# Ascend-Research/HeadPoseEstimation-WHENet

Hardware: AMD Instinct MI355X
Metric: head crops/sec (224x224) (higher is better)
Workload: dtype f16

## Files before the change

### headposeestimation-whenet_amd/csrc/capi.cpp

```cpp
#include <algorithm>
#include <chrono>
#include <cstdio>
#include <cstring>
#include <fstream>
#include <memory>
#include <mutex>
#include <new>
#include <exception>
#include <string>
#include <thread>
#include <utility>
#include <vector>

#include "engine.h"
#include "engine_internal.h"

constexpr int MAX_INFLIGHT_ENGINES = 4;
struct whenet_ctx {
    whenet::Engine* engine = nullptr;
    std::vector<whenet::Engine*> replicas;
    std::vector<char> snapshot;
    int device_id = 0, dtype = WHENET_F32;
    int inflight = 1;
    size_t next = 0;
// ... 1212 lines not shown
        std::memcpy(out, v, sizeof(v));
        return WHENET_OK;
    } catch (...) {
        return WHENET_EINVAL;
    }
}

int whenet_front2_static_check(int row, int field, int delta) {
    try {
        return whenet::front2_static_selftest(row, field, delta) == 0 ? WHENET_OK : WHENET_EINVAL;
    } catch (...) {
        return WHENET_EINVAL;
    }
}

int whenet_front_static_check(int row, int field, int delta) {
    try {
        return whenet::front_static_selftest(row, field, delta) == 0 ? WHENET_OK : WHENET_EINVAL;
    } catch (...) {
        return WHENET_EINVAL;
    }
}

int whenet_pw_static_check(int row, int field, int delta) {
    try {
        return whenet::pw_static_selftest(row, field, delta) == 0 ? WHENET_OK : WHENET_EINVAL;
    } catch (...) {
        return WHENET_EINVAL;
    }
}
// ... 21 lines not shown
```

### headposeestimation-whenet_amd/csrc/engine.cpp

```cpp
#include "engine_internal.h"

#include <mutex>

#include <algorithm>
#include <cstdlib>
#include <cmath>
#include <cstring>

namespace whenet {

using namespace detail;

void* Engine::upload_bytes(const void* p, size_t nbytes) {
    weight_allocs_.emplace_back();
    weight_allocs_.back().reset(nbytes);
    void* d = weight_allocs_.back().as<void>();
    if (nbytes) WHENET_HIP_CHECK(hipMemcpy(d, p, nbytes, hipMemcpyHostToDevice));
    return d;
}

template <typename T> T* Engine::upload(const std::vector<T>& v) {
    return static_cast<T*>(upload_bytes(v.data(), v.size() * sizeof(T)));
}

// ... 211 lines not shown
        WHENET_REQUIRE(split_ || value == 0, WHENET_EINVAL, "split_pw: the handle was not created as WHENET_F32S");
        split_pw_ = value != 0;
    } else if (key == "detector_dtype") {
        WHENET_REQUIRE(value == 0 || value == 1, WHENET_EINVAL, "detector_dtype must be 0 (binary16 storage, default) or 1 (float32)");
        const int dtype = value == 1 ? WHENET_F32 : WHENET_F16;
        WHENET_REQUIRE(det_ == nullptr || dtype == det_dtype_, WHENET_EINVAL,
                       "detector_dtype: a detector is attached and its weights were packed when it was loaded: set the option on a "
                       "handle without a detector, then load again");
        det_dtype_ = dtype;
        return;
    } else if (key == "host_pinned_max") {
        WHENET_REQUIRE(value >= 0 && value <= 4096, WHENET_EINVAL, "host_pinned_max must be 0..4096");
        sync();
        host_pinned_max_ = int(value);
        return;
    } else if (key == "se_fuse_tiny") {
        WHENET_REQUIRE(value >= 0 && value <= 64, WHENET_EINVAL, "se_fuse_tiny must be 0..64");
        se_fuse_tiny_ = int(value);
    } else if (key == "letterbox_cache") {
        WHENET_REQUIRE(value >= 1 && value <= 32, WHENET_EINVAL, "letterbox_cache must be 1..32");
        sync();
        lb_cache_.clear();
        lb_cache_cap_ = int(value);
        return;
    } else if (key == "jpeg_entropy") {
        WHENET_REQUIRE(value >= 0 && value <= 2, WHENET_EINVAL, "jpeg_entropy must be 0 (an interval per lane), 1 (segmented) or 2 (auto, default)");
        jpeg_entropy_ = int(value);
        return;
    } else if (key == "jpeg_seg_lanes") {
        WHENET_REQUIRE(value == 0 || value == 16 || value == 32 || value == 64, WHENET_EINVAL, "jpeg_seg_lanes must be 0 (default), 16, 32 or 64");
// ... 168 lines not shown
    } else {
        const DevBlock& c = blocks_[size_t(index)];
        const BlockSchedule cs = block_schedule(c);
        if (cs.use_mb7 || !cs.use_f7) return false;
        if (c.spec.has_skip() && c.project.K < 320) return false;
    }
    static constexpr bool WINS[17] = {false, false, false, false, false, false, false, false, false, false, false, false,
                                      true, true, true, true, true};
    return act_layout_ == 2 || (index <= 16 && WINS[index]);
}

bool Engine::front2_static(int index) const {
    static constexpr bool WINS[17] = {false, false, true, true, true, true, false, true, true, true, true, true, true,
                                      false, false, false, false};
    return front2_static_ && index >= 0 && index <= 16 && WINS[index];
}

bool Engine::pw_static(int index) const {
    static constexpr bool WINS[17] = {false, false, true, true, true, false, false, true, false, true, false, false, false,
                                      true, true, true, true};
    return pw_static_ && se_fuse_ == 1 && index >= 0 && index <= 16 && WINS[index];
}

bool Engine::front_static(int index) const {
    static constexpr bool WINS[17] = {false, false, false, false, false, false, true, false, false, false, false, false, false,
                                      false, false, false, false};
    return front_static_ && index >= 0 && index <= 16 && WINS[index];
}

void* Engine::enqueue_blocks(int first, int last, const View& v, void* cur, int n, hipStream_t s, LaunchRecorder* rec,
// ... 109 lines not shown
        fill_front_tiled(a, b);
        a.wep = b.expand.wp;
        a.wdt = b.dw.wt;
        if (fold == 2) {
            a.wep = d_fold12_w32_;
            a.be = fold12_pw_.bias;
            a.Cin = fold12_pw_.K;
            a.KSe = fold12_pw_.KS;
            a.NTe = fold12_pw_.NTILES;
            a.in_gate = static_cast<const float*>(v.gate);
        }
        a.xcd_grouped = xcd_grouped(1, n);
        a.plan = b.f2plan;
        a.plan.threads = front2_threads(b.f2plan, n);
        a.static_form = front2_static(sp.index);
        R(p + "/front", "front",
          kernel_name_front2(sp.k, sp.s, a.KSe, a.plan.threads, a.plan.xs, a.in_gate != nullptr, front2_static_row(a)).c_str(),
          bytes(a.Cin), flops(a.Cin), [&] { launch_front2(a, s); });
    } else if (bs.use_f2s) {
        Front2sArgs a{};
        fill_front_common(a, b, v, in, n);
        fill_front_tiled(a, b);
        a.weps = b.expand.wps;
        a.wdt = b.dw.wts;
        a.KSe = b.expand.KSs;
        a.wsi = b.expand.wsi;
        a.wsi_d = b.dw.wts_wsi;
        a.tm = b.f2s_tm;
        a.plan = b.f2splan;
        R(p + "/front", "front", kernel_name_front2s(sp.k, sp.s, a.KSe, a.plan.threads, a.tm, false).c_str(), bytes(a.Cin),
          flops(a.Cin), [&] { launch_front2s(a, s); });
    } else {
// ... 594 lines not shown
```

### headposeestimation-whenet_amd/csrc/engine.h

```cpp
#pragma once

#include <deque>
#include <map>
#include <memory>
#include <string>
#include <tuple>
#include <utility>
#include <vector>

#include "common.h"
#include "kernels.h"
#include "snapshot.h"

namespace whenet {

template <typename H, hipError_t (*Destroy)(H)>
class Owned {
  public:
    Owned() = default;
    Owned(Owned&& o) noexcept : h_(o.h_) { o.h_ = nullptr; }
    ~Owned() { reset(); }
    void reset() {
        if (h_) (void)Destroy(h_);
        h_ = nullptr;
// ... 344 lines not shown
                         hipStream_t s, LaunchRecorder* rec, bool in_blocked, bool out_blocked);
    template <typename A> void fill_front_common(A& a, const DevBlock& b, const View& v, const void* in, int n) const;
    Head7Args head7_args(const void* x, float* feat, int n) const;
    PwArgs head_pw_args(const void* x, void* out, int n) const { return pw_args(head_, x, out, n * 49, 49, ACT_SWISH); }
    void* enqueue_blocks(int first, int last, const View& v, void* cur, int n, hipStream_t s, LaunchRecorder* rec,
                         bool b1_dw_done = false);
    bool stem_fuse_active() const;
    bool fold12_active() const;
    bool head_fused() const;
    bool heads_split_active() const;
    void launch_heads_stage(const HeadsArgs& h, const View& v, hipStream_t s);
    bool act_blocked(int index) const;
    bool front_static(int index) const;
    bool pw_static(int index) const;
    bool front2_static(int index) const;
    int act_layout_ = 1;
    struct BlockSchedule {
        bool fused = false, use_f2 = false, use_f2s = false, use_f7 = false, se_in_front = false, se_fused = false, se_mfma = false;
        bool use_mb7 = false;
        int se_ntiles = 1, se_chunks = 1;
    };
    BlockSchedule block_schedule(const DevBlock& b, int n = 0) const;
    int se_fuse_tiny_ = 0;
    int f2s_mask_ = -1;
    bool single_stage_call_ = false;
    bool range_call_ = false;
    int lanes_for(int n, int want) const;
    template <typename F> void for_each_lane(int n, int lanes, hipStream_t s, F&& body);
    void enqueue_lanes(const uint8_t* d_in, int n, Results out, hipStream_t s, int want = 0);
    void run_forward(const uint8_t* d_in, int n, Results out, hipStream_t s, int want = 0);
// ... 71 lines not shown
    int se_fuse_ = 1;
    int front_impl_ = 1;
    bool poison_ = false;
    bool head_fuse_ = true;
    bool front7_ = true;
    bool mb7_ = false;
    int xcd_map_ = 7;
    bool xcd_always_ = false;
    bool xcd_grouped(int bit, int n) const {
        return (xcd_map_ & bit) != 0 && (xcd_always_ || n >= 128);
    }
    bool stem_fuse_ = true;
    bool front_static_ = true;
    bool pw_static_ = true;
    bool front2_static_ = true;
    bool fold12_ = true;
    int lanes_ = 2;
    bool lane_graphs_ = false;
    int min_lane_crops_ = 16;
    int host_lanes_ = 2;
    Stream stream_, copy_stream_;
    std::vector<Stream> lane_streams_;
    std::vector<Event> join_ev_;
    Event fork_ev_;
    hipDeviceProp_t prop_{};
    int64_t params_backbone_ = 0, params_heads_ = 0;
    int n_tensors_ = 0;

    std::vector<DeviceBuffer> weight_allocs_;
    float *d_lut_ = nullptr, *d_stem_w_ = nullptr, *d_stem_b_ = nullptr;
// ... 59 lines not shown
```

### headposeestimation-whenet_amd/csrc/front2.hip

```cpp
#include "device_math.h"
#include "kernels.h"
#include "stamps.h"

#include <atomic>
#include <cstdlib>
#include <string>
#include <vector>

namespace whenet {

namespace {

constexpr int RL = 7;

__device__ __forceinline__ int fdiv2(int q, float rinv) { return int((float(q) + 0.5f) * rinv); }

struct F2Params {
    const half_t* x;
    const half_t* wep;
    const float* be;
    const half_t* wdt;
    const float* bd;
    half_t* out;
    float* rpart;
    const float* w1t;
    const float* in_gate;
    int H, Ho, Cin, Cexp, pad, NTe;
    int CC, TH, TXG, tiles_x, EH, EWp, RP, CP;
    int off_stage, off_red, off_sum;
    int R, RPse;
    int ntiles, chunks, n, xcd;
};

struct Tuned2 { int k, s, H, Cexp, CC, TH, TXG, xs, use, threads; };
constexpr Tuned2 TUNED2[] = {
#include "front2_tuned.inc"
};
constexpr int NTUNED2 = int(sizeof(TUNED2) / sizeof(TUNED2[0]));

struct F2Shape {
    int H, Ho, Cin, Cexp, pad, NTe;
    int CC, TH, TXG, tiles_x, tiles_y, EH, EWp, RP, CP;
    int off_stage, off_red, off_sum;
    int R, RPse;
    int ntiles, chunks;
    int k, s, xs, threads, KS, gated, lds_bytes;
};

constexpr int cdiv(int a, int b) { return (a + b - 1) / b; }

constexpr F2Shape f2_static_shape(int row) {
    const Tuned2 t = TUNED2[row];
    F2Shape g{};
// ... 38 lines not shown
#pragma unroll
    for (int qq = 0; qq < 4; ++qq) {
        if (!EDGE || (drd[qq] < nr_left && dcd[qq] < ng_left)) {
            const float2v y0 = swish2(float2v{acc[4 * qq], acc[4 * qq + 1]});
            const float2v y1 = swish2(float2v{acc[4 * qq + 2], acc[4 * qq + 3]});
            half4 o;
            o[0] = half_t(y0[0]);
            o[1] = half_t(y0[1]);
            o[2] = half_t(y1[0]);
            o[3] = half_t(y1[1]);
            *reinterpret_cast<half4*>(ep + eoff[qq]) = o;
        }
    }
}

template <int K, int S, int KS, int NTHR, int XS, bool GATED, int ROW>
__device__ __forceinline__ void front2_body(const F2Params p) {
    constexpr F2Shape sg = f2_static_shape(ROW < 0 ? 0 : ROW);
    static_assert(ROW < 0 || (sg.k == K && sg.s == S && sg.KS == KS && sg.threads == NTHR && sg.xs == XS && (sg.gated != 0) == GATED),
                  "front2: the static plan belongs to another instantiation");
#define GEO(f) (ROW >= 0 ? sg.f : p.f)
    constexpr bool ONE_TILE = ROW >= 0 && sg.CC <= 32;
    constexpr int NCH = (3 * S + K + XS + 3) / 4;
    constexpr int NER = (RL - 1) * S + K;
    constexpr int NWAVE = NTHR / 64;
    constexpr int PF = KS <= 7 ? KS : 6;

    extern __shared__ __attribute__((aligned(16))) unsigned char smem[];
    unsigned char* E = smem;

// ... 347 lines not shown
                    const int c = q + 4 * i;
                    if (c < ccur) accr = fmaf(s_sum[c], w1v[i], accr);
                }
                for (int c = q + 4 * W1V; c < ccur; c += 4) accr = fmaf(s_sum[c], wrow[c], accr);
            }
            const float pair = accr + quad_xor1(accr);
            const float tot = pair + quad_xor2(pair);
            if (q == 0)
                p.rpart[((size_t(b) * GEO(ntiles) + tile) * GEO(chunks) + chunk) * GEO(RPse) + jo] = (jo < GEO(R)) ? tot : 0.0f;
        }
    }
    STAMP(6);
}
#undef GEO

template <int K, int S, int KS, int NTHR, int XS, bool GATED>
__global__ __launch_bounds__(NTHR) void whenet_front2_kernel(const F2Params p) {
    front2_body<K, S, KS, NTHR, XS, GATED, -1>(p);
}

template <int K, int S, int KS, int NTHR, int XS, bool GATED, int ROW>
__global__ __launch_bounds__(NTHR) void whenet_front2_static_kernel(const F2Params p) {
    front2_body<K, S, KS, NTHR, XS, GATED, ROW>(p);
}

}

namespace {

constexpr bool f2_has_static(int row) { return TUNED2[row].use != 0; }

const char* f2_static_mismatch(const F2Shape& g, const Front2Args& a) {
    const Front2Plan& pl = a.plan;
    struct Field { const char* name; long long want, got; };
    const Field fields[] = {
        {"H", g.H, a.H}, {"Ho", g.Ho, a.Ho}, {"Cin", g.Cin, a.Cin}, {"Cexp", g.Cexp, a.Cexp}, {"pad", g.pad, a.pad}, {"NTe", g.NTe, a.NTe},
        {"CC", g.CC, pl.CC}, {"TH", g.TH, pl.TH}, {"TXG", g.TXG, pl.TXG}, {"tiles_x", g.tiles_x, pl.tiles_x}, {"tiles_y", g.tiles_y, pl.tiles_y},
        {"EH", g.EH, pl.EH}, {"EWp", g.EWp, pl.EWp}, {"RP", g.RP, pl.RP}, {"CP", g.CP, pl.CP},
// ... 20 lines not shown
        if (!f2_has_static(r)) continue;
        const F2Shape g = f2_static_shape(r);
        if (g.k == a.k && g.s == a.s && g.H == a.H && g.Ho == a.Ho && g.Cin == a.Cin && g.Cexp == a.Cexp && g.pad == a.pad && g.NTe == a.NTe &&
            g.KS == a.KSe && g.R == a.R && (g.gated != 0) == (a.in_gate != nullptr) && g.CC == a.plan.CC && g.TH == a.plan.TH &&
            g.TXG == a.plan.TXG && g.xs == a.plan.xs && g.threads == a.plan.threads)
            return r;
    }
    return -1;
}

void front2_static_check(int row, const Front2Args& a) {
    WHENET_REQUIRE(row >= 0 && row < NTUNED2 && f2_has_static(row), WHENET_EINVAL, "front2: no static form for this row of the plan table");
    f2_static_require(f2_static_shape(row), a);
}

int front2_static_selftest(int row, int field, int delta) {
    WHENET_REQUIRE(row >= 0 && row < NTUNED2 && f2_has_static(row), WHENET_EINVAL, "front2: no static form for this row of the plan table");
    WHENET_REQUIRE(field >= -1 && field < int(sizeof(F2Shape) / sizeof(int)), WHENET_EINVAL, "front2: no such field");
    F2Shape g = f2_static_shape(row);
    Front2Args a{};
    a.k = g.k;  a.s = g.s;  a.H = g.H;  a.Ho = g.Ho;  a.Cin = g.Cin;  a.Cexp = g.Cexp;  a.pad = g.pad;  a.NTe = g.NTe;  a.KSe = g.KS;  a.R = g.R;
    a.in_gate = g.gated ? reinterpret_cast<const float*>(&g) : nullptr;
    a.plan = make_front2_plan(g.k, g.s, g.Ho, g.Cexp, TUNED2[row].CC, TUNED2[row].TH, TUNED2[row].TXG, TUNED2[row].threads, TUNED2[row].xs);
    if (field >= 0) reinterpret_cast<int*>(&g)[field] += delta;
    f2_static_require(g, a);
    return 0;
}

namespace {

struct OncePerDevice {
    std::atomic<bool> done[64];
    OncePerDevice() { for (auto& d : done) d.store(false, std::memory_order_relaxed); }
};

template <int K, int S, int KS, int NTHR, int XS = 0, bool GATED = false, int ROW = -1>
void launch_f2(const Front2Args& a, hipStream_t stream) {
    const auto kernel = [] {
        if constexpr (ROW >= 0) return &whenet_front2_static_kernel<K, S, KS, NTHR, XS, GATED, ROW>;
        else return &whenet_front2_kernel<K, S, KS, NTHR, XS, GATED>;
    }();
    const Front2Plan& pl = a.plan;
    F2Params p{};
    p.x = static_cast<const half_t*>(a.x);
    p.wep = static_cast<const half_t*>(a.wep);
    p.be = a.be;
    p.wdt = static_cast<const half_t*>(a.wdt);
    p.bd = a.bd;
    p.out = static_cast<half_t*>(a.out);
    p.rpart = a.rpart;
    p.w1t = a.w1t;
    p.in_gate = a.in_gate;
    p.H = a.H;  p.Ho = a.Ho;  p.Cin = a.Cin;  p.Cexp = a.Cexp;  p.pad = a.pad;  p.NTe = a.NTe;
    p.CC = pl.CC;  p.TH = pl.TH;  p.TXG = pl.TXG;  p.tiles_x = pl.tiles_x;
    p.EH = pl.EH;  p.EWp = pl.EWp;  p.RP = pl.RP;  p.CP = pl.CP;
    p.off_stage = pl.off_stage;  p.off_red = pl.off_red;  p.off_sum = pl.off_sum;
    p.R = a.R;  p.RPse = (a.R + 3) & ~3;
    p.ntiles = pl.tiles_x * pl.tiles_y;  p.chunks = pl.chunks;  p.n = a.n;  p.xcd = a.xcd_grouped ? 1 : 0;
    WHENET_REQUIRE(pl.lds_bytes <= 160 * 1024, WHENET_EINVAL, "front2: the tile plan needs more than 160 KB of LDS");
    static OncePerDevice attr;
    int dev = 0;
    WHENET_HIP_CHECK(hipGetDevice(&dev));
    if (dev >= 0 && dev < 64 && !attr.done[dev].load(std::memory_order_acquire)) {
        if constexpr (ROW >= 0) front2_static_check(ROW, a);
        WHENET_HIP_CHECK(hipFuncSetAttribute(reinterpret_cast<const void*>(kernel), hipFuncAttributeMaxDynamicSharedMemorySize, 160 * 1024));
        attr.done[dev].store(true, std::memory_order_release);
    }
    hipLaunchKernelGGL(kernel, dim3(unsigned(pl.tiles_x * pl.tiles_y) * unsigned(pl.chunks) * unsigned(a.n)), dim3(NTHR),
                       pl.lds_bytes, stream, p);
    WHENET_HIP_CHECK(hipGetLastError());
}

void launch_f2_static(int row, const Front2Args& a, hipStream_t stream) {
    switch (row) {
        case 0: launch_f2<3, 2, 2, 512, 0, true, 0>(a, stream); break;
        case 1: launch_f2<3, 1, 2, 256, 0, false, 1>(a, stream); break;
        case 2: launch_f2<5, 2, 2, 256, 0, false, 2>(a, stream); break;
        case 3: launch_f2<5, 1, 3, 256, 0, false, 3>(a, stream); break;
        case 5: launch_f2<3, 1, 5, 256, 0, false, 5>(a, stream); break;
        case 6: launch_f2<5, 1, 5, 256, 0, false, 6>(a, stream); break;
        case 7: launch_f2<5, 1, 7, 256, 0, false, 7>(a, stream); break;
        case 8: launch_f2<5, 2, 7, 256, 0, false, 8>(a, stream); break;
        default: throw Error(WHENET_EINVAL, "front2: no static form for this row of the plan table");
    }
}

template <int NTHR>
void launch_f2_shape(const Front2Args& a, hipStream_t stream) {
// ... 113 lines not shown

void launch_front2(const Front2Args& a, hipStream_t stream) {
    WHENET_REQUIRE(a.KSe == ceil_div(a.Cin, 16), WHENET_EINVAL, "front2: k-steps do not match Cin");
    WHENET_REQUIRE(a.in_gate == nullptr || (a.k == 3 && a.s == 2 && a.KSe == 2 && a.Cin == 32), WHENET_EINVAL,
                   "front2: the gated-input form exists for the 3x3 / stride-2 / Cin = 32 shape only");
    Front2Args b = a;
    if (b.plan.threads != 256) {
        b.plan = make_front2_plan(a.k, a.s, a.Ho, a.Cexp, a.plan.CC, a.plan.TH, a.plan.TXG, a.plan.threads, a.plan.xs);
    }
    const int row = front2_static_row(b);
    if (row >= 0) launch_f2_static(row, b, stream);
    else if (b.plan.threads == 512) launch_f2_shape<512>(b, stream);
    else launch_f2_shape<256>(b, stream);
}

std::string kernel_name_front2(int k, int s, int kse, int threads, int xs, bool gated, int static_row) {
    return std::string(static_row >= 0 ? "whenet_front2_static_kernel<" : "whenet_front2_kernel<") + std::to_string(k) + ", " +
           std::to_string(s) + ", " + std::to_string(kse) + ", " + std::to_string(threads) + ", " + std::to_string(xs) + ", " +
           (gated ? "true" : "false") + (static_row >= 0 ? ", " + std::to_string(static_row) : std::string()) + ">";
}

}
```

### headposeestimation-whenet_amd/csrc/kernels.h

```cpp
#pragma once

#include <string>
#include <vector>

#include "common.h"
#include "overlay_host.h"
#include "jpeg_host.h"
#include "jpeg_dec_host.h"
#include "jpeg_dec_seg_host.h"

namespace whenet {

struct StemArgs {
    const uint8_t* in;
    void* out;
    const float* w;
    const float* bias;
    const float* lut;
    int n;
    const float* in_f32 = nullptr;
};
void launch_stem(const StemArgs& a, int dtype, hipStream_t stream);

struct DwPlan {
// ... 201 lines not shown
struct Front2Args {
    const void* x;
    const void* wep;
    const float* be;
    const void* wdt;
    const float* bd;
    void* out;
    float* rpart;
    const float* w1t;
    const float* in_gate;
    int R;
    int k, s, H, Ho, Cin, Cexp, pad, KSe, NTe, n;
    Front2Plan plan;
    bool xcd_grouped = false;
    bool static_form = false;
};
void launch_front2(const Front2Args& a, hipStream_t stream);
std::string kernel_name_front2(int k, int s, int kse, int threads, int xs, bool gated, int static_row = -1);
int front2_static_row(const Front2Args& a);
void front2_static_check(int row, const Front2Args& a);
int front2_static_selftest(int row, int field, int delta);

struct Front2sArgs {
    const void* x;
    const void* weps;
    const float* be;
    const void* wdt;
    const float* bd;
    void* out;
    float* rpart;
    const float* w1t;
    int R;
    int k, s, H, Ho, Cin, Cexp, pad, KSe, NTe, n;
    float wsi = 1.0f;
    float wsi_d = 1.0f;
    int tm = 2;
// ... 340 lines not shown
```

### headposeestimation-whenet_amd/whenet_hip/_lib.py

```python
from __future__ import annotations

import ctypes as C
import os
from typing import Optional

import numpy as np

ABI_VERSION = 6
F32, F16, F32S = 0, 1, 2
OK, ENOENT, EIO, ENOMEM, ENODEV, EINVAL, EFORMAT, EHIP = 0, -2, -5, -12, -19, -22, -74, -1000
EOVERFLOW = -75
MAX_INFLIGHT = 4

_HERE = os.path.dirname(os.path.abspath(__file__))
LIB_PATH = os.path.join(_HERE, "..", "lib", "libwhenet_hip.so")


class Info(C.Structure):
    _fields_ = [("abi_version", C.c_int32), ("dtype", C.c_int32), ("device_id", C.c_int32),
                ("compute_units", C.c_int32), ("params_backbone", C.c_int64),
                ("params_heads", C.c_int64), ("n_tensors", C.c_int32),
                ("n_kernels_per_forward", C.c_int32), ("macs_per_crop", C.c_int64),
                ("arena_bytes", C.c_int64), ("capacity", C.c_int32), ("graph_enabled", C.c_int32),
                ("device_name", C.c_char * 64), ("arch", C.c_char * 32)]
# ... 112 lines not shown
    "whenet_jpeg_decode_segmented_planes_host": (C.c_int, [_P, C.c_int64, C.POINTER(_P), _P, C.c_int, C.c_int, _P, _P]),
    "whenet_op_jpeg_decode_ex": (C.c_int, [_P, _P, C.c_int64, C.POINTER(SurfaceC), C.c_int, C.c_int, C.c_int, _P, _P]),
    "whenet_jpeg_decode_counters": (C.c_int, [_P, C.POINTER(C.c_int64 * 4)]),
    "whenet_jpeg_seg_dc_scan_host": (C.c_int, [_P, C.c_int64, C.c_int, _P]),
    "whenet_frame_begin_jpeg": (C.c_int, [_P, _P, C.c_int64, C.c_int, C.POINTER(C.c_int), _P]),
    "whenet_profile": (C.c_int, [_P, _P, C.c_int, C.c_int, C.POINTER(LaunchStat), C.c_int, C.POINTER(C.c_int)]),
    "whenet_op_stem": (C.c_int, [_P, _P, C.c_int, _P]),
    "whenet_op_block": (C.c_int, [_P, C.c_int, _P, C.c_int, _P, _P, _P, _P]),
    "whenet_op_block_range": (C.c_int, [_P, C.c_int, C.c_int, _P, C.c_int, _P]),
    "whenet_op_head": (C.c_int, [_P, _P, C.c_int, _P, _P, _P, _P]),
    "whenet_op_decode": (C.c_int, [_P, _P, C.c_int, _P, _P]),
    "whenet_block_spec": (C.c_int, [C.c_int, C.POINTER(C.c_int32 * 8)]),
    "whenet_dw_plan": (C.c_int, [C.c_int, C.c_int, C.POINTER(C.c_int32 * 12)]),
    "whenet_front_plan": (C.c_int, [C.c_int, C.c_int, C.POINTER(C.c_int32 * 12)]),
    "whenet_front2_static_check": (C.c_int, [C.c_int, C.c_int, C.c_int]),
    "whenet_pw_static_check": (C.c_int, [C.c_int, C.c_int, C.c_int]),
    "whenet_front_static_check": (C.c_int, [C.c_int, C.c_int, C.c_int]),
    "whenet_device_alloc": (C.c_int, [_P, C.c_size_t, C.POINTER(_P)]),
    "whenet_device_free": (C.c_int, [_P, _P]),
    "whenet_memcpy_h2d": (C.c_int, [_P, _P, _P, C.c_size_t]),
    "whenet_memcpy_d2h": (C.c_int, [_P, _P, _P, C.c_size_t]),
}
EXPORTS = tuple(_PROTOS)

_lib: Optional[C.CDLL] = None


def load() -> C.CDLL:
    global _lib
    if _lib is not None:
# ... 1170 lines not shown
```

### include/whenet_hip.h

```cpp
#ifndef WHENET_HIP_H
#define WHENET_HIP_H

#include <stddef.h>
#include <stdint.h>

#ifdef __cplusplus
extern "C" {
#endif

#define WHENET_ABI_VERSION 6
#define WHENET_API __attribute__((visibility("default")))

#define WHENET_OK        0
#define WHENET_ENOENT   (-2)
#define WHENET_EIO      (-5)
#define WHENET_ENOMEM   (-12)
#define WHENET_ENODEV   (-19)
#define WHENET_EINVAL   (-22)
#define WHENET_EFORMAT  (-74)
#define WHENET_EHIP     (-1000)

#define WHENET_F32 0
#define WHENET_F16 1
#define WHENET_F32S 2
// ... 271 lines not shown
WHENET_API int whenet_op_block(whenet_t* h, int index, const float* in, int n,
                    float* expand_out, float* dw_out, float* gate, float* out);
WHENET_API int whenet_op_block_range(whenet_t* h, int first, int last, const float* in, int n, float* out);
WHENET_API int whenet_op_head(whenet_t* h, const float* in, int n,
                   float* feat, float* logits, float* ypr, int32_t* argmax);
WHENET_API int whenet_op_decode(whenet_t* h, const float* logits, int n, float* ypr, int32_t* argmax);

WHENET_API int whenet_block_spec(int index, int32_t out[8]);

WHENET_API int whenet_dw_plan(int dtype, int index, int32_t out[12]);

WHENET_API int whenet_front_plan(int dtype, int index, int32_t out[12]);

WHENET_API int whenet_front2_static_check(int row, int field, int delta);

WHENET_API int whenet_pw_static_check(int row, int field, int delta);

WHENET_API int whenet_front_static_check(int row, int field, int delta);

WHENET_API int whenet_device_alloc(whenet_t* h, size_t nbytes, void** d_ptr);
WHENET_API int whenet_device_free(whenet_t* h, void* d_ptr);
WHENET_API int whenet_memcpy_h2d(whenet_t* h, void* d_dst, const void* src, size_t nbytes);
WHENET_API int whenet_memcpy_d2h(whenet_t* h, void* dst, const void* d_src, size_t nbytes);

#ifdef __cplusplus
}
#endif
#endif
```

Baseline: 184,900.

## Add walk form of static front2 kernel covering several tile rows per block

Adds a variant of the static front2 (expand+depthwise) kernel in which each workgroup walks down several consecutive tile rows, loading the channel tile's weight fragments once. Optionally it keeps the halo rows of the expanded tile in registers between steps so they are not recomputed. The grid shrinks by the walk depth. By default it is enabled for layers 2 and 3 when launches have at least 128 or 256 crops. This trades parallelism (fewer blocks) for less redundant weight loading and halo recomputation, adding a lot of new code and more register pressure.

```diff
diff --git a/headposeestimation-whenet_amd/csrc/capi.cpp b/headposeestimation-whenet_amd/csrc/capi.cpp
--- a/headposeestimation-whenet_amd/csrc/capi.cpp
+++ b/headposeestimation-whenet_amd/csrc/capi.cpp
@@ -1250,6 +1250,32 @@
     }
 }
 
+int whenet_front2_walk_check(int row, int d_depth, int d_units) {
+    try {
+        return whenet::front2_walk_selftest(row, d_depth, d_units) > 1 ? WHENET_OK : WHENET_EINVAL;
+    } catch (...) {
+        return WHENET_EINVAL;
+    }
+}
+
+int whenet_front2_walk_option(long long value) { return whenet::front2_walk_option_valid(value) ? WHENET_OK : WHENET_EINVAL; }
+
+int whenet_front2_walk_depth(int row, int32_t out[2]) {
+    if (out == nullptr) return WHENET_EINVAL;
+    try {
+        const auto blocks = whenet::make_blocks();
+        out[0] = whenet::front2_walk_depth(row);
+        out[1] = 0;
+        if (row >= 0 && row <= 3) {
+            const whenet::BlockSpec& b = blocks[size_t(row + 1)];
+            out[1] = whenet::plan_front2(b.k, b.s, b.h_in, b.h_out, b.cexp()).tiles_y;
+        }
+        return WHENET_OK;
+    } catch (...) {
+        return WHENET_EINVAL;
+    }
+}
+
 int whenet_front_static_check(int row, int field, int delta) {
     try {
         return whenet::front_static_selftest(row, field, delta) == 0 ? WHENET_OK : WHENET_EINVAL;
diff --git a/headposeestimation-whenet_amd/csrc/engine.cpp b/headposeestimation-whenet_amd/csrc/engine.cpp
--- a/headposeestimation-whenet_amd/csrc/engine.cpp
+++ b/headposeestimation-whenet_amd/csrc/engine.cpp
@@ -249,6 +249,10 @@
         sync();
         host_pinned_max_ = int(value);
         return;
+    } else if (key == "front2_walk") {
+        WHENET_REQUIRE(front2_walk_option_valid(value), WHENET_EINVAL,
+                       "front2_walk must be 0 (never), 1 (per layer, launches of at least 128 crops: default) or 2 (every layer that has a walk form, at any launch size)");
+        front2_walk_ = int(value);
     } else if (key == "se_fuse_tiny") {
         WHENET_REQUIRE(value >= 0 && value <= 64, WHENET_EINVAL, "se_fuse_tiny must be 0..64");
         se_fuse_tiny_ = int(value);
@@ -447,6 +451,16 @@
     static constexpr bool WINS[17] = {false, false, true, true, true, true, false, true, true, true, true, true, true,
                                       false, false, false, false};
     return front2_static_ && index >= 0 && index <= 16 && WINS[index];
+}
+
+bool Engine::front2_walk(int index, int n) const {
+#ifndef WHENET_FRONT2_WALK_FROM
+#define WHENET_FRONT2_WALK_FROM 128, 256, 0, 0
+#endif
+    static constexpr int FROM[17] = {0, 0, WHENET_FRONT2_WALK_FROM, 0, 0, 0, 0, 0, 0, 0, 0, 0, 0, 0};
+    if (front2_walk_ == 0 || !front2_static(index)) return false;
+    if (front2_walk_ == 2) return true;
+    return index <= 16 && FROM[index] > 0 && n >= FROM[index];
 }
 
 bool Engine::pw_static(int index) const {
@@ -586,8 +600,10 @@
         a.plan = b.f2plan;
         a.plan.threads = front2_threads(b.f2plan, n);
         a.static_form = front2_static(sp.index);
+        a.walk = front2_walk(sp.index, n);
+        const int f2row = front2_static_row(a);
         R(p + "/front", "front",
-          kernel_name_front2(sp.k, sp.s, a.KSe, a.plan.threads, a.plan.xs, a.in_gate != nullptr, front2_static_row(a)).c_str(),
+          kernel_name_front2(sp.k, sp.s, a.KSe, a.plan.threads, a.plan.xs, a.in_gate != nullptr, f2row, a.walk ? front2_walk_depth(f2row) : 1).c_str(),
           bytes(a.Cin), flops(a.Cin), [&] { launch_front2(a, s); });
     } else if (bs.use_f2s) {
         Front2sArgs a{};
diff --git a/headposeestimation-whenet_amd/csrc/engine.h b/headposeestimation-whenet_amd/csrc/engine.h
--- a/headposeestimation-whenet_amd/csrc/engine.h
+++ b/headposeestimation-whenet_amd/csrc/engine.h
@@ -382,6 +382,7 @@
     bool front_static(int index) const;
     bool pw_static(int index) const;
     bool front2_static(int index) const;
+    bool front2_walk(int index, int n) const;
     int act_layout_ = 1;
     struct BlockSchedule {
         bool fused = false, use_f2 = false, use_f2s = false, use_f7 = false, se_in_front = false, se_fused = false, se_mfma = false;
@@ -483,6 +484,7 @@
     bool front_static_ = true;
     bool pw_static_ = true;
     bool front2_static_ = true;
+    int front2_walk_ = 1;
     bool fold12_ = true;
     int lanes_ = 2;
     bool lane_graphs_ = false;
diff --git a/headposeestimation-whenet_amd/csrc/front2.hip b/headposeestimation-whenet_amd/csrc/front2.hip
--- a/headposeestimation-whenet_amd/csrc/front2.hip
+++ b/headposeestimation-whenet_amd/csrc/front2.hip
@@ -37,6 +37,15 @@
 #include "front2_tuned.inc"
 };
 constexpr int NTUNED2 = int(sizeof(TUNED2) / sizeof(TUNED2[0]));
+
+struct F2Walk { int depth, keep, ahead; };
+#ifndef WHENET_F2_WALK_TABLE
+#define WHENET_F2_WALK_TABLE {4, 0, 1}, {2, 1, 1}, {2, 1, 1}, {2, 1, 1}
+#endif
+constexpr F2Walk WALK2[NTUNED2] = {
+    WHENET_F2_WALK_TABLE,
+    {1, 0, 0}, {1, 0, 0}, {1, 0, 0}, {1, 0, 0}, {1, 0, 0}, {1, 0, 0}, {1, 0, 0},
+};
 
 struct F2Shape {
     int H, Ho, Cin, Cexp, pad, NTe;
@@ -105,6 +114,23 @@
     }
 }
 
+struct F2Strips { int scl, nsc, g_lo; };
+constexpr F2Strips f2_static_strips(int row) {
+    const F2Shape g = f2_static_shape(row);
+    F2Strips r{0, 0, 0};
+    for (int txi = 0; txi < g.tiles_x; ++txi) {
+        const int ix0 = txi * g.TXG * 4 * g.s - g.pad - g.xs;
+        const int ex_lo = ix0 < 0 ? -ix0 : 0, ex_hi = (ix0 + g.EWp < g.H) ? g.EWp : g.H - ix0;
+        const int g_lo = ex_lo >> 2, NG = ((ex_hi + 3) >> 2) - g_lo;
+        const int scl = NG <= 2 ? 1 : (NG <= 4 ? 2 : 3), nsc = (NG + (1 << scl) - 1) >> scl;
+        if (txi == 0) r = F2Strips{scl, nsc, g_lo};
+        if (scl != r.scl) r.scl = -1;
+        if (nsc != r.nsc) r.nsc = -1;
+        if (g_lo != r.g_lo) r.g_lo = -1;
+    }
+    return r;
+}
+
 template <int K, int S, int KS, int NTHR, int XS, bool GATED, int ROW>
 __device__ __forceinline__ void front2_body(const F2Params p) {
     constexpr F2Shape sg = f2_static_shape(ROW < 0 ? 0 : ROW);
@@ -482,14 +508,478 @@
 }
 #undef GEO
 
+template <int K, int S, int KS, int NTHR, int XS, bool GATED, int ROW, int WALK>
+__device__ __forceinline__ void front2_walk_body(const F2Params p) {
+    static_assert(ROW >= 0 && WALK >= 2, "front2: the walk is a form of the static kernels");
+    constexpr F2Shape sg = f2_static_shape(ROW);
+    static_assert(sg.k == K && sg.s == S && sg.KS == KS && sg.threads == NTHR && sg.xs == XS && (sg.gated != 0) == GATED,
+                  "front2: the static plan belongs to another instantiation");
+#define GEO(f) (sg.f)
+    constexpr bool ONE_TILE = sg.CC <= 32;
+    constexpr F2Walk wk = WALK2[ROW];
+    static_assert(WALK == wk.depth && sg.tiles_y % WALK == 0, "front2: the walk's depth is the table's and divides the tile rows");
+    static_assert(ONE_TILE, "front2: the walk loads the weight fragments of ONE channel tile, once");
+    constexpr bool KEEP = wk.keep != 0, AHEAD = wk.ahead != 0;
+    constexpr int HR = K - S;
+    constexpr int NCH = (3 * S + K + XS + 3) / 4;
+    constexpr int NER = (RL - 1) * S + K;
+    constexpr int NWAVE = NTHR / 64;
+    constexpr int PF = KS <= 7 ? KS : 6;
+
+    extern __shared__ __attribute__((aligned(16))) unsigned char smem[];
+    unsigned char* E = smem;
+
+    const int tid = threadIdx.x;
+    const int lane = tid & 63;
+    const int wave = __builtin_amdgcn_readfirstlane(tid >> 6);
+    const int g = lane >> 5, lm = lane & 31;
+    int b, tile, chunk;
+    xcd_front(int(blockIdx.x), GEO(ntiles) / WALK, GEO(chunks), p.n, p.xcd != 0, b, tile, chunk);
+    int tyi = tile / GEO(tiles_x);
+    const int txi = tile - tyi * GEO(tiles_x);
+    tyi *= WALK;
+    tile = tyi * GEO(tiles_x) + txi;
+    const int c0 = chunk * GEO(CC);
+    const int ccur = (ROW >= 0 && sg.Cexp % sg.CC == 0) ? sg.CC
+                                                        : ((GEO(Cexp) - c0 < GEO(CC)) ? (GEO(Cexp) - c0) : GEO(CC));
+    const int H = GEO(H), Cin = GEO(Cin), RP = GEO(RP), CP = GEO(CP);
+    int oy0, iy0, ez_lo, er_lo, er_hi, NR, nsr, nstrip, ntask, t_begin, t_end;
+    oy0 = tyi * GEO(TH);
+    const int ox0 = txi * GEO(TXG) * 4;
+    iy0 = oy0 * S - GEO(pad);
+    const int ix0 = ox0 * S - GEO(pad) - XS;
+
+    er_lo = ez_lo = iy0 < 0 ? -iy0 : 0;
+    er_hi = (iy0 + GEO(EH) < H) ? GEO(EH) : H - iy0;
+    const int ex_lo = ix0 < 0 ? -ix0 : 0, ex_hi = (ix0 + GEO(EWp) < H) ? GEO(EWp) : H - ix0;
+    constexpr F2Strips sx = f2_static_strips(ROW);
+    const int g_lo = sx.g_lo >= 0 ? sx.g_lo : ex_lo >> 2, g_hi = (ex_hi + 3) >> 2;
+    const int NG = g_hi - g_lo;
+    NR = er_hi - er_lo;
+    const int SCL = sx.scl >= 0 ? sx.scl : (NG <= 2 ? 1 : (NG <= 4 ? 2 : 3)), SC = 1 << SCL, SRL = 3 - SCL, SR = 1 << SRL;
+    const int nsc = sx.nsc >= 0 ? sx.nsc : (NG + SC - 1) >> SCL;
+    nsr = (NR + SR - 1) >> SRL;
+    const int ntile = (ccur + 31) >> 5;
+    nstrip = nsc * nsr;
+    ntask = nstrip * ntile;
+
+    const unsigned char* xb = reinterpret_cast<const unsigned char*>(p.x + size_t(b) * H * H * Cin);
+    const half8* wf0 = reinterpret_cast<const half8*>(p.wep) + size_t(c0 >> 5) * 64 + lane;
+
+    const int ua = lm >> 2;
+    const int pixoff_a = (ua >> SCL) * H + 4 * (ua & (SC - 1)) + (lm & 3);
+    int eoff[4], drd[4], dcd[4];
+#pragma unroll
+    for (int qq = 0; qq < 4; ++qq) {
+        const int u = 2 * qq + g;
+        drd[qq] = u >> SCL;
+        dcd[qq] = u & (SC - 1);
+        eoff[qq] = drd[qq] * RP + dcd[qq] * 8;
+    }
+    const int npix1 = H * H - 1;
+    const unsigned cin2 = unsigned(Cin) * 2u;
+    auto a_offset = [&](int rb, int cbk) -> unsigned {
+        const int pb = (iy0 + er_lo + (rb << SRL)) * H + ix0 + 4 * (g_lo + (cbk << SCL));
+        int pl = pb + pixoff_a;
+        pl = pl < 0 ? 0 : (pl > npix1 ? npix1 : pl);
+        return __umul24(unsigned(pl), cin2) + unsigned(g) * 16u;
+    };
+
+    t_begin = (wave * ntask) / NWAVE;
+    t_end = ((wave + 1) * ntask) / NWAVE;
+    auto set_tile = [&]() {
+        oy0 = tyi * GEO(TH);
+        iy0 = oy0 * S - GEO(pad);
+        ez_lo = iy0 < 0 ? -iy0 : 0;
+        er_hi = (iy0 + GEO(EH) < H) ? GEO(EH) : H - iy0;
+        er_lo = KEEP ? HR : ez_lo;
+        NR = er_hi - er_lo;
+        nsr = (NR + SR - 1) >> SRL;
+        nstrip = nsc * nsr;
+        ntask = nstrip * ntile;
+        t_begin = (wave * ntask) / NWAVE;
+        t_end = ((wave + 1) * ntask) / NWAVE;
+    };
+#ifndef WHENET_F2_RING
+#define WHENET_F2_RING 1
+#endif
+    constexpr int D = WHENET_F2_RING;
+    half8 w[KS], aq[D][PF];
+    float bias_cur = 0.f;
+    float16v bias16;
+    float4v gq[GATED ? KS : 1][2];
+    if constexpr (GATED) {
+        const float* gp = reinterpret_cast<const float*>(p.in_gate) + size_t(b) * Cin + g * 8;
+#pragma unroll
+        for (int ks = 0; ks < KS; ++ks) {
+            gq[ks][0] = *reinterpret_cast<const float4v*>(gp + ks * 16);
+            gq[ks][1] = *reinterpret_cast<const float4v*>(gp + ks * 16 + 4);
+        }
+    }
+    auto load_w = [&](int tl) {
+#pragma unroll
+        for (int ks = 0; ks < KS; ++ks) {
+            if constexpr (GATED) {
+                const float* wq = reinterpret_cast<const float*>(p.wep) + ((size_t(ks) * GEO(NTe) + (c0 >> 5) + tl) * 64 + lane) * 8;
+                const float4v lo = *reinterpret_cast<const float4v*>(wq) * gq[ks][0];
+                const float4v hi = *reinterpret_cast<const float4v*>(wq + 4) * gq[ks][1];
+#pragma unroll
+                for (int e = 0; e < 4; ++e) {
+                    w[ks][e] = half_t(lo[e]);
+                    w[ks][4 + e] = half_t(hi[e]);
+                }
+            } else {
+                w[ks] = wf0[(size_t(ks) * GEO(NTe) + tl) * 64];
+            }
+        }
+        const int ch = tl * 32 + lm;
+        bias_cur = (ch < ccur) ? p.be[c0 + ch] : 0.f;
+#pragma unroll
+        for (int r = 0; r < 16; ++r) bias16[r] = bias_cur;
+    };
+    const bool ktail = (Cin & 15) != 0 && g == 1;
+    auto load_a = [&](half8 (&a)[PF], unsigned off, int ks0) {
+#pragma unroll
+        for (int u = 0; u < PF; ++u)
+            if (ks0 + u < KS) a[u] = *reinterpret_cast<const half8*>(xb + off + (ks0 + u) * 32);
+    };
+    auto zero_ktail = [&](half8 (&a)[PF], int ks0) {
+#pragma unroll
+        for (int u = 0; u < PF; ++u)
+            if (ks0 + u == KS - 1 && ktail) a[u] = half8{0, 0, 0, 0, 0, 0, 0, 0};
+    };
+    STAMP(0);
+    int tl = 0, rb = 0, cbk = 0;
+    int ti = t_begin, rbi = 0, cbki = 0;
+    unsigned aoffq[D];
+    auto issue = [&](int slot) {
+        if (ti < t_end) {
+            aoffq[slot] = a_offset(rbi, cbki);
+            load_a(aq[slot], aoffq[slot], 0);
+        }
+        ++ti;
+        if (++cbki == nsc) {
+            cbki = 0;
+            if (++rbi == nsr) rbi = 0;
+        }
+    };
+    const bool fix_l = ex_lo > 0, fix_r = GEO(EWp) > ex_hi;
+    auto prime = [&]() {
+        ti = t_begin;
+        if (t_begin < t_end) {
+            tl = 0;
+            const int st = t_begin;
+            rb = __builtin_amdgcn_readfirstlane(st / nsc);
+            cbk = st - rb * nsc;
+            rbi = rb;
+            cbki = cbk;
+#pragma unroll
+            for (int d = 0; d < D; ++d) issue(d);
+        }
+    };
+    auto next_tile = [&]() {
+        ++tyi;
+        tile += GEO(tiles_x);
+        set_tile();
+        prime();
+    };
+    load_w(0);
+    prime();
+    half4 A[K][NCH];
+    float bdv = 0.f;
+    constexpr int W1V = 16;
+    float w1v[W1V];
+    constexpr int HP_ROW = sg.RP / 8, HP_ALL = sg.CC * HR * HP_ROW, NHP = KEEP ? cdiv(HP_ALL, NTHR) : 1;
+    half4 hv[NHP];
+
+  auto one_tile = [&](const int wt) __attribute__((always_inline)) {
+    {
+        asm volatile("" : "+v"(bias_cur));
+#pragma unroll
+        for (int r = 0; r < 16; ++r) bias16[r] = bias_cur;
+    }
+#define TSTAMP(i) do { if (wt == WALK - 1) STAMP(i); } while (0)
+    TSTAMP(7);
+    {
+        const int nz = ez_lo + (GEO(EH) - er_hi);
+        if (nz > 0) {
+            const float r_nz = __builtin_amdgcn_rcpf(float(nz));
+            for (int pr = tid; pr < ccur * nz; pr += NTHR) {
+                const int c = fdiv2(pr, r_nz), hr = pr - c * nz;
+                const int er = hr < ez_lo ? hr : er_hi + (hr - ez_lo);
+                unsigned char* rowp = E + c * CP + ((c >> 3) & 1) * 8 + er * RP;
+                for (int q = 0; q < RP; q += 8) *reinterpret_cast<half4*>(rowp + q) = half4{0, 0, 0, 0};
+            }
+        }
+    }
+
+    TSTAMP(1);
+    for (int t0 = t_begin; t0 < t_end; t0 += D) {
+#pragma unroll
+      for (int d = 0; d < D; ++d) {
+        const int t = t0 + d;
+        if (t >= t_end) break;
+        float16v acc;
+        zero_ktail(aq[d], 0);
+        acc = __builtin_amdgcn_mfma_f32_32x32x16_f16(aq[d][0], w[0], bias16, 0, 0, 0);
+#pragma unroll
+        for (int u = 1; u < PF; ++u) acc = __builtin_amdgcn_mfma_f32_32x32x16_f16(aq[d][u], w[u], acc, 0, 0, 0);
+#pragma unroll
+        for (int ks = PF; ks < KS; ks += PF) {
+            load_a(aq[d], aoffq[d], ks);
+            zero_ktail(aq[d], ks);
+#pragma unroll
+            for (int u = 0; u < PF; ++u)
+                if (ks + u < KS) acc = __builtin_amdgcn_mfma_f32_32x32x16_f16(aq[d][u], w[ks + u], acc, 0, 0, 0);
+        }
+        const int ch = tl * 32 + lm;
+        unsigned char* ep = E + ch * CP + ((ch >> 3) & 1) * 8 + (er_lo + (rb << SRL)) * RP + (g_lo + (cbk << SCL)) * 8;
+        unsigned char* ep0 = ep;
+        const int nr_left = NR - (rb << SRL), ng_left = NG - (cbk << SCL), cbk_this = cbk;
+        const float bias = bias_cur;
+        int tln = tl;
+        if (++cbk == nsc) {
+            cbk = 0;
+            if (++rb == nsr) {
+                rb = 0;
+                if (!ONE_TILE) ++tln;
+            }
+        }
+        issue(d);
+        if (!ONE_TILE && t + 1 < t_end && tln != tl) load_w(tln);
+        tl = tln;
+        if (ch < ccur) {
+            if (nr_left >= SR && ng_left >= SC) expand_store<false>(acc, bias, ep, eoff, drd, dcd, nr_left, ng_left);
+            else expand_store<true>(acc, bias, ep, eoff, drd, dcd, nr_left, ng_left);
+        }
+        if (ch < ccur) {
+            if (fix_l && cbk_this == 0) {
+#pragma unroll
+                for (int dd = 0; dd < 2; ++dd) {
+                    const int dr = g + 2 * dd;
+                    if (dr < SR && dr < nr_left) {
+                        half_t* rowp = reinterpret_cast<half_t*>(ep0 + dr * RP) - 4 * g_lo;
+#pragma unroll
+                        for (int q = 0; q < 4; ++q)
+                            if (q < ex_lo) rowp[q] = half_t(0);
+                    }
+                }
+            }
+            if (fix_r && cbk_this == nsc - 1) {
+#pragma unroll
+                for (int dd = 0; dd < 2; ++dd) {
+                    const int dr = g + 2 * dd;
+                    if (dr < SR && dr < nr_left) {
+                        half_t* rowp = reinterpret_cast<half_t*>(ep0 + dr * RP) - 4 * (g_lo + cbk_this * SC) + ex_hi;
+#pragma unroll
+                        for (int q = 0; q < 8; ++q)
+                            if (ex_hi + q < GEO(EWp)) rowp[q] = half_t(0);
+                    }
+                }
+            }
+        }
+      }
+    }
+
+    TSTAMP(2);
+    const int oy0_t = oy0, tile_t = tile;
+    int tid_t = tid, b_t = b;
+    int has_w1_t = p.w1t != nullptr ? 1 : 0;
+    asm volatile("" : "+v"(tid_t), "+s"(b_t), "+v"(has_w1_t));
+    has_w1_t = __builtin_amdgcn_readfirstlane(has_w1_t);
+    const bool has_w1 = has_w1_t != 0;
+    const int lane_t = tid_t & 63;
+    if constexpr (AHEAD) {
+        if (wt + 1 < WALK) next_tile();
+    }
+    const int ncb = (ccur + 15) >> 4;
+    const int ncol = (GEO(TH) / RL) * GEO(TXG), ncq = (ncol + 3) >> 2, nitem = ncb * ncq;
+    const float r_txg = __builtin_amdgcn_rcpf(float(GEO(TXG)));
+    const int i_begin = (wave * nitem) / NWAVE, i_end = ((wave + 1) * nitem) / NWAVE;
+    const int cl = lane_t >> 2, j = lane_t & 3;
+    auto load_taps = [&](int cb) {
+        const half4* src = reinterpret_cast<const half4*>(p.wdt) + (size_t((c0 >> 4) + cb) * K * NCH) * 64 + lane_t;
+#pragma unroll
+        for (int ky = 0; ky < K; ++ky)
+#pragma unroll
+            for (int ch = 0; ch < NCH; ++ch) A[ky][ch] = src[(ky * NCH + ch) * 64];
+        bdv = p.bd[c0 + cb * 16 + cl];
+    };
+    int cb = 0, cq = 0;
+    if (i_begin < i_end) {
+        cb = __builtin_amdgcn_readfirstlane(i_begin / ncq);
+        cq = i_begin - cb * ncq;
+        load_taps(cb);
+    }
+    lds_barrier();
+    TSTAMP(3);
+    {
+        const int jo = tid_t >> 2, q = tid_t & 3;
+#pragma unroll
+        for (int i = 0; i < W1V; ++i) w1v[i] = 0.f;
+        if (has_w1 && wave * 16 < GEO(RPse)) {
+            const float* wrow = p.w1t + size_t(jo < GEO(R) ? jo : GEO(R) - 1) * GEO(Cexp) + c0;
+#pragma unroll
+            for (int i = 0; i < W1V; ++i) {
+                const int c = q + 4 * i;
+                w1v[i] = wrow[c < ccur ? c : ccur - 1];
+            }
+        }
+    }
+    unsigned char* stg = smem + GEO(off_stage) + wave * 2048;
+    float* s_red = reinterpret_cast<float*>(smem + GEO(off_red));
+    float* s_sum = reinterpret_cast<float*>(smem + GEO(off_sum));
+    const int jP = (lane_t >> 1) & 3, iP = (lane_t >> 3) & 3, hP = lane_t & 1, rP = lane_t >> 5;
+    unsigned char* outb = reinterpret_cast<unsigned char*>(p.out + size_t(b_t) * GEO(Ho) * GEO(Ho) * GEO(Cexp));
+    const unsigned row_bytes = unsigned(GEO(Ho)) * unsigned(GEO(Cexp)) * 2u;
+
+    for (int it = i_begin; it < i_end; ++it) {
+        const int col = cq * 4 + j;
+        const int colc = col < ncol ? col : ncol - 1;
+        const int seg = fdiv2(colc, r_txg), xgl = colc - seg * GEO(TXG);
+        const int c = cb * 16 + cl;
+        const unsigned char* bp = E + c * CP + ((c >> 3) & 1) * 8 + (seg * RL * S) * RP + xgl * (8 * S);
+        float4v acc[RL];
+        const float4v bd4 = float4v{bdv, bdv, bdv, bdv};
+        bool started[RL];
+#pragma unroll
+        for (int r = 0; r < RL; ++r) started[r] = false;
+#pragma unroll
+        for (int er = 0; er < NER; ++er) {
+            half4 bv[NCH];
+#pragma unroll
+            for (int ch = 0; ch < NCH; ++ch) bv[ch] = *reinterpret_cast<const half4*>(bp + er * RP + ch * 8);
+#pragma unroll
+            for (int ky = 0; ky < K; ++ky) {
+                const int d = er - ky;
+                if (d >= 0 && d % S == 0 && d / S < RL) {
+#pragma unroll
+                    for (int ch = 0; ch < NCH; ++ch) {
+                        acc[d / S] = __builtin_amdgcn_mfma_f32_4x4x4f16(A[ky][ch], bv[ch], started[d / S] ? acc[d / S] : bd4, 0, 0, 0);
+                        started[d / S] = true;
+                    }
+                }
+            }
+        }
+        const int cb_this = cb, cq_this = cq;
+        if (++cq == ncq) {
+            cq = 0;
+            ++cb;
+            if (it + 1 < i_end) load_taps(cb);
+        }
+        const bool okc = col < ncol;
+        const int oxb = ox0 + 4 * xgl;
+        float m[4];
+#pragma unroll
+        for (int i = 0; i < 4; ++i) m[i] = (okc && oxb + i < GEO(Ho)) ? 1.f : 0.f;
+        const int colP = cq_this * 4 + jP;
+        const int colPc = colP < ncol ? colP : ncol - 1;
+        const int segP = fdiv2(colPc, r_txg), xglP = colPc - segP * GEO(TXG);
+        const int oxP = ox0 + 4 * xglP + iP;
+        const bool okP = colP < ncol && oxP < GEO(Ho);
+        const unsigned obase = (__umul24(unsigned(oy0_t + segP * RL + rP), unsigned(GEO(Ho))) + unsigned(oxP)) * unsigned(GEO(Cexp)) * 2u +
+                               unsigned(c0 + cb_this * 16 + hP * 8) * 2u;
+        float2v sum2 = {0.f, 0.f};
+        const float2v m01 = {m[0], m[1]}, m23 = {m[2], m[3]};
+        unsigned char* sw = stg + j * 32 + cl * 2;
+#pragma unroll
+        for (int half = 0; half < 2; ++half) {
+            const int r0 = half * 4, nr = half ? 3 : 4;
+#pragma unroll
+            for (int r = 0; r < nr; ++r) {
+                const float2v y01 = swish2(float2v{acc[r0 + r][0], acc[r0 + r][1]});
+                const float2v y23 = swish2(float2v{acc[r0 + r][2], acc[r0 + r][3]});
+                sum2 = y01 * m01 + sum2;
+                sum2 = y23 * m23 + sum2;
+                *reinterpret_cast<half_t*>(sw + (r * 4 + 0) * 128) = half_t(y01[0]);
+                *reinterpret_cast<half_t*>(sw + (r * 4 + 1) * 128) = half_t(y01[1]);
+                *reinterpret_cast<half_t*>(sw + (r * 4 + 2) * 128) = half_t(y23[0]);
+                *reinterpret_cast<half_t*>(sw + (r * 4 + 3) * 128) = half_t(y23[1]);
+            }
+            wave_lds_sync();
+#pragma unroll
+            for (int pp = 0; pp < 2; ++pp) {
+                const int rl = 2 * pp + rP;
+                const half8 v = *reinterpret_cast<const half8*>(stg + (pp * 64 + lane_t) * 16);
+                if (okP && rl < nr) *reinterpret_cast<half8*>(outb + obase + unsigned(r0 + 2 * pp) * row_bytes) = v;
+            }
+            wave_lds_sync();
+        }
+        float sum = sum2[0] + sum2[1];
+        sum += quad_xor1(sum);
+        sum += quad_xor2(sum);
+        if (j == 0) s_red[cq_this * GEO(CC) + c] = sum;
+    }
+    TSTAMP(4);
+    lds_barrier();
+    TSTAMP(5);
+    if constexpr (KEEP) {
+        if (wt + 1 < WALK) {
+#pragma unroll
+            for (int i = 0; i < NHP; ++i) {
+                const int q = tid_t + i * NTHR;
+                const int c = q / (HR * HP_ROW), r = q - c * (HR * HP_ROW);
+                if (q < HP_ALL && c < ccur) hv[i] = *reinterpret_cast<const half4*>(E + c * CP + ((c >> 3) & 1) * 8 + GEO(TH) * S * RP + r * 8);
+            }
+        }
+    }
+
+    if (tid_t < ccur) {
+        float t = 0.0f;
+        for (int q = 0; q < ncq; ++q) t += s_red[q * GEO(CC) + tid_t];
+        if (!has_w1) p.rpart[(size_t(b_t) * GEO(ntiles) + tile_t) * GEO(Cexp) + c0 + tid_t] = t;
+        s_sum[tid_t] = t;
+    }
+    if (has_w1) {
+        lds_barrier();
+        const int jo = tid_t >> 2, q = tid_t & 3;
+        if (jo < GEO(RPse)) {
+            float accr = 0.0f;
+            if (jo < GEO(R)) {
+                const float* wrow = p.w1t + size_t(jo) * GEO(Cexp) + c0;
+#pragma unroll
+                for (int i = 0; i < W1V; ++i) {
+                    const int c = q + 4 * i;
+                    if (c < ccur) accr = fmaf(s_sum[c], w1v[i], accr);
+                }
+                for (int c = q + 4 * W1V; c < ccur; c += 4) accr = fmaf(s_sum[c], wrow[c], accr);
+            }
+            const float pair = accr + quad_xor1(accr);
+            const float tot = pair + quad_xor2(pair);
+            if (q == 0)
+                p.rpart[((size_t(b_t) * GEO(ntiles) + tile_t) * GEO(chunks) + chunk) * GEO(RPse) + jo] = (jo < GEO(R)) ? tot : 0.0f;
+        }
+    }
+    TSTAMP(6);
+    if (wt + 1 < WALK) {
+        if constexpr (KEEP) {
+            if (!has_w1) lds_barrier();
+#pragma unroll
+            for (int i = 0; i < NHP; ++i) {
+                const int q = tid_t + i * NTHR;
+                const int c = q / (HR * HP_ROW), r = q - c * (HR * HP_ROW);
+                if (q < HP_ALL && c < ccur) *reinterpret_cast<half4*>(E + c * CP + ((c >> 3) & 1) * 8 + r * 8) = hv[i];
+            }
+        }
+        if constexpr (!AHEAD) next_tile();
+    }
+  };
+    one_tile(0);
+#pragma unroll 1
+    for (int wt = 1; wt < WALK; ++wt) one_tile(wt);
+#undef TSTAMP
+}
+#undef GEO
+
 template <int K, int S, int KS, int NTHR, int XS, bool GATED>
 __global__ __launch_bounds__(NTHR) void whenet_front2_kernel(const F2Params p) {
     front2_body<K, S, KS, NTHR, XS, GATED, -1>(p);
 }
 
-template <int K, int S, int KS, int NTHR, int XS, bool GATED, int ROW>
+template <int K, int S, int KS, int NTHR, int XS, bool GATED, int ROW, int WALK = 1>
 __global__ __launch_bounds__(NTHR) void whenet_front2_static_kernel(const F2Params p) {
-    front2_body<K, S, KS, NTHR, XS, GATED, ROW>(p);
+    if constexpr (WALK == 1) front2_body<K, S, KS, NTHR, XS, GATED, ROW>(p);
+    else front2_walk_body<K, S, KS, NTHR, XS, GATED, ROW, WALK>(p);
 }
 
 }
@@ -540,14 +1030,42 @@
     f2_static_require(f2_static_shape(row), a);
 }
 
+int front2_walk_depth(int row) { return row >= 0 && row < NTUNED2 && f2_has_static(row) ? WALK2[row].depth : 1; }
+
+namespace {
+
+void f2_walk_require(int row, int depth, int units, const Front2Args& a) {
+    const Front2Plan& pl = a.plan;
+    WHENET_REQUIRE(depth > 1 && depth == front2_walk_depth(row) && pl.tiles_y % depth == 0, WHENET_EINVAL,
+                   "front2: the walk's depth is not the table's, or does not divide the runtime plan's tile rows");
+    WHENET_REQUIRE(units == pl.tiles_x * (pl.tiles_y / depth) && units * depth == pl.tiles_x * pl.tiles_y, WHENET_EINVAL,
+                   "front2: the walk's grid differs from the runtime plan's tiles");
+}
+
+Front2Args f2_selftest_args(int row, F2Shape& g) {
+    Front2Args a{};
+    a.k = g.k;  a.s = g.s;  a.H = g.H;  a.Ho = g.Ho;  a.Cin = g.Cin;  a.Cexp = g.Cexp;  a.pad = g.pad;  a.NTe = g.NTe;  a.KSe = g.KS;  a.R = g.R;
+    a.in_gate = g.gated ? reinterpret_cast<const float*>(&g) : nullptr;
+    a.plan = make_front2_plan(g.k, g.s, g.Ho, g.Cexp, TUNED2[row].CC, TUNED2[row].TH, TUNED2[row].TXG, TUNED2[row].threads, TUNED2[row].xs);
+    return a;
+}
+
+}
+
+int front2_walk_selftest(int row, int d_depth, int d_units) {
+    WHENET_REQUIRE(row >= 0 && row < NTUNED2 && f2_has_static(row) && WALK2[row].depth > 1, WHENET_EINVAL, "front2: no walk for this row of the plan table");
+    F2Shape g = f2_static_shape(row);
+    const Front2Args a = f2_selftest_args(row, g);
+    const int depth = WALK2[row].depth;
+    f2_walk_require(row, depth + d_depth, g.ntiles / depth + d_units, a);
+    return depth;
+}
+
 int front2_static_selftest(int row, int field, int delta) {
     WHENET_REQUIRE(row >= 0 && row < NTUNED2 && f2_has_static(row), WHENET_EINVAL, "front2: no static form for this row of the plan table");
     WHENET_REQUIRE(field >= -1 && field < int(sizeof(F2Shape) / sizeof(int)), WHENET_EINVAL, "front2: no such field");
     F2Shape g = f2_static_shape(row);
-    Front2Args a{};
-    a.k = g.k;  a.s = g.s;  a.H = g.H;  a.Ho = g.Ho;  a.Cin = g.Cin;  a.Cexp = g.Cexp;  a.pad = g.pad;  a.NTe = g.NTe;  a.KSe = g.KS;  a.R = g.R;
-    a.in_gate = g.gated ? reinterpret_cast<const float*>(&g) : nullptr;
-    a.plan = make_front2_plan(g.k, g.s, g.Ho, g.Cexp, TUNED2[row].CC, TUNED2[row].TH, TUNED2[row].TXG, TUNED2[row].threads, TUNED2[row].xs);
+    const Front2Args a = f2_selftest_args(row, g);
     if (field >= 0) reinterpret_cast<int*>(&g)[field] += delta;
     f2_static_require(g, a);
     return 0;
@@ -560,10 +1078,10 @@
     OncePerDevice() { for (auto& d : done) d.store(false, std::memory_order_relaxed); }
 };
 
-template <int K, int S, int KS, int NTHR, int XS = 0, bool GATED = false, int ROW = -1>
+template <int K, int S, int KS, int NTHR, int XS = 0, bool GATED = false, int ROW = -1, int WALK = 1>
 void launch_f2(const Front2Args& a, hipStream_t stream) {
     const auto kernel = [] {
-        if constexpr (ROW >= 0) return &whenet_front2_static_kernel<K, S, KS, NTHR, XS, GATED, ROW>;
+        if constexpr (ROW >= 0) return &whenet_front2_static_kernel<K, S, KS, NTHR, XS, GATED, ROW, WALK>;
         else return &whenet_front2_kernel<K, S, KS, NTHR, XS, GATED>;
     }();
     const Front2Plan& pl = a.plan;
@@ -589,15 +1107,25 @@
     WHENET_HIP_CHECK(hipGetDevice(&dev));
     if (dev >= 0 && dev < 64 && !attr.done[dev].load(std::memory_order_acquire)) {
         if constexpr (ROW >= 0) front2_static_check(ROW, a);
+        if constexpr (WALK > 1) f2_walk_require(ROW, WALK, f2_static_shape(ROW).ntiles / WALK, a);
         WHENET_HIP_CHECK(hipFuncSetAttribute(reinterpret_cast<const void*>(kernel), hipFuncAttributeMaxDynamicSharedMemorySize, 160 * 1024));
         attr.done[dev].store(true, std::memory_order_release);
     }
-    hipLaunchKernelGGL(kernel, dim3(unsigned(pl.tiles_x * pl.tiles_y) * unsigned(pl.chunks) * unsigned(a.n)), dim3(NTHR),
+    hipLaunchKernelGGL(kernel, dim3(unsigned(pl.tiles_x * pl.tiles_y / WALK) * unsigned(pl.chunks) * unsigned(a.n)), dim3(NTHR),
                        pl.lds_bytes, stream, p);
     WHENET_HIP_CHECK(hipGetLastError());
 }
 
 void launch_f2_static(int row, const Front2Args& a, hipStream_t stream) {
+    if (a.walk && front2_walk_depth(row) > 1) {
+        switch (row) {
+            case 0: launch_f2<3, 2, 2, 512, 0, true, 0, WALK2[0].depth>(a, stream); return;
+            case 1: launch_f2<3, 1, 2, 256, 0, false, 1, WALK2[1].depth>(a, stream); return;
+            case 2: launch_f2<5, 2, 2, 256, 0, false, 2, WALK2[2].depth>(a, stream); return;
+            case 3: launch_f2<5, 1, 3, 256, 0, false, 3, WALK2[3].depth>(a, stream); return;
+            default: break;
+        }
+    }
     switch (row) {
         case 0: launch_f2<3, 2, 2, 512, 0, true, 0>(a, stream); break;
         case 1: launch_f2<3, 1, 2, 256, 0, false, 1>(a, stream); break;
@@ -741,10 +1269,11 @@
     else launch_f2_shape<256>(b, stream);
 }
 
-std::string kernel_name_front2(int k, int s, int kse, int threads, int xs, bool gated, int static_row) {
+std::string kernel_name_front2(int k, int s, int kse, int threads, int xs, bool gated, int static_row, int walk) {
     return std::string(static_row >= 0 ? "whenet_front2_static_kernel<" : "whenet_front2_kernel<") + std::to_string(k) + ", " +
            std::to_string(s) + ", " + std::to_string(kse) + ", " + std::to_string(threads) + ", " + std::to_string(xs) + ", " +
-           (gated ? "true" : "false") + (static_row >= 0 ? ", " + std::to_string(static_row) : std::string()) + ">";
-}
-
-}
+           (gated ? "true" : "false") + (static_row >= 0 ? ", " + std::to_string(static_row) : std::string()) +
+           (static_row >= 0 && walk > 1 ? ", " + std::to_string(walk) : std::string()) + ">";
+}
+
+}
diff --git a/headposeestimation-whenet_amd/csrc/kernels.h b/headposeestimation-whenet_amd/csrc/kernels.h
--- a/headposeestimation-whenet_amd/csrc/kernels.h
+++ b/headposeestimation-whenet_amd/csrc/kernels.h
@@ -239,12 +239,16 @@
     Front2Plan plan;
     bool xcd_grouped = false;
     bool static_form = false;
+    bool walk = false;
 };
 void launch_front2(const Front2Args& a, hipStream_t stream);
-std::string kernel_name_front2(int k, int s, int kse, int threads, int xs, bool gated, int static_row = -1);
+std::string kernel_name_front2(int k, int s, int kse, int threads, int xs, bool gated, int static_row = -1, int walk = 1);
 int front2_static_row(const Front2Args& a);
 void front2_static_check(int row, const Front2Args& a);
 int front2_static_selftest(int row, int field, int delta);
+int front2_walk_depth(int row);
+inline bool front2_walk_option_valid(long long v) { return v >= 0 && v <= 2; }
+int front2_walk_selftest(int row, int d_depth, int d_units);
 
 struct Front2sArgs {
     const void* x;
diff --git a/headposeestimation-whenet_amd/whenet_hip/_lib.py b/headposeestimation-whenet_amd/whenet_hip/_lib.py
--- a/headposeestimation-whenet_amd/whenet_hip/_lib.py
+++ b/headposeestimation-whenet_amd/whenet_hip/_lib.py
@@ -150,6 +150,9 @@
     "whenet_dw_plan": (C.c_int, [C.c_int, C.c_int, C.POINTER(C.c_int32 * 12)]),
     "whenet_front_plan": (C.c_int, [C.c_int, C.c_int, C.POINTER(C.c_int32 * 12)]),
     "whenet_front2_static_check": (C.c_int, [C.c_int, C.c_int, C.c_int]),
+    "whenet_front2_walk_check": (C.c_int, [C.c_int, C.c_int, C.c_int]),
+    "whenet_front2_walk_option": (C.c_int, [C.c_longlong]),
+    "whenet_front2_walk_depth": (C.c_int, [C.c_int, C.POINTER(C.c_int32 * 2)]),
     "whenet_pw_static_check": (C.c_int, [C.c_int, C.c_int, C.c_int]),
     "whenet_front_static_check": (C.c_int, [C.c_int, C.c_int, C.c_int]),
     "whenet_device_alloc": (C.c_int, [_P, C.c_size_t, C.POINTER(_P)]),
diff --git a/include/whenet_hip.h b/include/whenet_hip.h
--- a/include/whenet_hip.h
+++ b/include/whenet_hip.h
@@ -309,6 +309,12 @@
 
 WHENET_API int whenet_front2_static_check(int row, int field, int delta);
 
+WHENET_API int whenet_front2_walk_check(int row, int d_depth, int d_units);
+
+WHENET_API int whenet_front2_walk_option(long long value);
+
+WHENET_API int whenet_front2_walk_depth(int row, int32_t out[2]);
+
 WHENET_API int whenet_pw_static_check(int row, int field, int delta);
 
 WHENET_API int whenet_front_static_check(int row, int field, int delta);
```

New measurement: 184,600. Within noise of the previous version (-0.1%).
